# LordLiang/DrawingSpinUp

Hardware: AMD Instinct MI355X
Metric: drawings/sec end-to-end (512x512, 6 views, 24 frames) (higher is better)
Workload: dtype f16 (diffusion) / f16 table + f32 MLP (NSR) / f32 (stage-1 deformable convolutions, IS-Net, contour) / f32 with bf16 x 3 products (stage-2 convolutions; the reference: cuDNN TF32)

## Files before the change

### drawingspinup_amd/csrc/nsr_driver.hip

```cpp
#include "common.h"
#include "adamw_dev.h"

#include <math.h>
#include <string.h>

#include <mutex>
#include <vector>

namespace {

constexpr int N_GEO = 64 * 23 + 64 + 13 * 64 + 13;
constexpr int N_TEX = 64 * 16 + 64 + 64 * 64 + 64 + 3 * 64 + 3;
constexpr int N_SMALL = (64 * 23 + 64 + 64) + (13 * 64 + 13 + 13) + N_TEX + 1;

__device__ __forceinline__ uint4 philox(uint4 c, uint2 k) {
#pragma unroll
  for (int i = 0; i < 10; ++i) {
    const uint32_t hi0 = __umulhi(0xD2511F53u, c.x), lo0 = 0xD2511F53u * c.x;
    const uint32_t hi1 = __umulhi(0xCD9E8D57u, c.z), lo1 = 0xCD9E8D57u * c.z;
    c = make_uint4(hi1 ^ c.y ^ k.x, lo1, hi0 ^ c.w ^ k.y, lo0);
    k.x += 0x9E3779B9u;
    k.y += 0xBB67AE85u;
  }
  return c;
// ... 681 lines not shown
    tex_red.base = L.g_tex;
    have_tex_red = true;
  } else {
    DSU_HIP(hipMemsetAsync(L.d_feat_all, 0, (size_t)(2 * n_r) * 13 * sizeof(float), s));
  }
  DSU_TRY(dsu_sample_losses(L.a_sdf, L.a_grad, n_s, n_r, c.lambda_eikonal, c.lambda_sparsity,
                            c.sparsity_scale, c.lambda_smooth, 1 | 2, L.d_sdf_all, L.d_grad_all,
                            terms + 4, s));
  float* gg = L.g_geo;
  DSU_TRY(mark(d, 1, s));
  DSU_TRY(dsu_sdf_fd_bwd_sorted_fold(&c.grid, a->table_img, &mlp, pts, perm, n_all, c.radius, a->eps,
                                     a->active_levels, L.d_sdf_all, L.d_grad_all, L.d_feat_all, nullptr,
                                     a->table_grad, gg, gg + 64 * 23, gg + 64 * 23 + 64,
                                     gg + 64 * 23 + 64 + 13 * 64, L.sdf_ws, L.sdf_ws_bytes,
                                     L.enc_cache, d->gate, have_tex_red ? &tex_red : nullptr, s));
  DSU_TRY(mark(d, 1, s));
  if (d->timing) { d->work[1] += alg_bytes; d->flops[1] += bwd_flops; }
  DSU_TRY(launch_small_update(d, a, 1, s));
  d->last_step = a->step;
  guard.ok = true;
  return DSU_OK;
}

int dsu_nsr_driver_occ_refresh(dsu_nsr_driver* d, const dsu_occgrid_refresh_args* args,
                               void* main_stream) {
  if (!d || !args) return DSU_EINVAL;
  if (!d->initialised) return DSU_EUNSUP;
  const dsu_nsr_driver_cfg& c = d->cfg;
  DSU_HIP(hipStreamSynchronize(d->side));
  for (int k = 0; k < 3; ++k) d->pf_valid[k] = false;
  dsu_occgrid_refresh_args a = *args;
  const dsu_sdf_mlp mlp{d->L.w0_eff, c.b0, d->L.w1_eff, c.b1};
  a.grid = &c.grid;
  a.mlp = &mlp;
  a.inv_s = d->L.inv_s;
  a.aabb = d->aabb;
  a.seed = c.seed;
  a.radius = c.radius;
  a.render_step_size = c.render_step_size;
  return dsu_occgrid_refresh(&a, main_stream);
}

int dsu_nsr_driver_timing(dsu_nsr_driver* d, int32_t enable) {
  if (!d) return DSU_EINVAL;
  for (int f = 0; f < 2; ++f) {
    for (hipEvent_t e : d->ev[f]) (void)hipEventDestroy(e);
// ... 35 lines not shown
```

### drawingspinup_amd/nsr/encoding.py

```python
import torch
import torch.nn as nn

from .. import ops


class _EncodeFn(torch.autograd.Function):
    @staticmethod
    def forward(ctx, x, params, enc, active):
        ctx.save_for_backward(x)
        ctx.enc, ctx.active = enc, active
        return ops.hashgrid_encode_fwd(enc.cfg, enc.table_f16(), x, active)

    @staticmethod
    def backward(ctx, dout):
        (x,) = ctx.saved_tensors
        g = ops.hashgrid_encode_bwd(ctx.enc.cfg, x, dout.float(), ctx.active)
        return None, g, None, None


_INIT_CACHE = {}


class Encoding(nn.Module):
    def __init__(self, n_input_dims, encoding_config, seed=1337, dtype=None):
# ... 53 lines not shown
    def forward(self, x):
        return _EncodeFn.apply(x.float().contiguous(), self.params, self, self.active_levels)


class ProgressiveBandHashGrid(nn.Module):

    def __init__(self, in_channels, config):
        super().__init__()
        self.n_input_dims = in_channels
        encoding_config = dict(config)
        encoding_config["otype"] = "HashGrid"
        self.encoding = Encoding(in_channels, encoding_config)
        self.n_output_dims = self.encoding.n_output_dims
        self.n_level = config["n_levels"]
        self.n_features_per_level = config["n_features_per_level"]
        self.start_level, self.start_step, self.update_steps = \
            config["start_level"], config["start_step"], config["update_steps"]
        self.current_level = self.start_level
        self.encoding.active_levels = self.current_level

    def forward(self, x):
        return self.encoding(x).float()

    def update_step(self, epoch, global_step):
        self.current_level = min(
            self.start_level + max(global_step - self.start_step, 0) // self.update_steps,
            self.n_level)
        self.encoding.active_levels = self.current_level
```

### drawingspinup_amd/nsr/model.py

```python
import math

import torch
import torch.nn as nn
import torch.nn.functional as F

from .. import ops
from .encoding import ProgressiveBandHashGrid
from .render import (ContractionType, OccupancyGrid, accumulate_along_rays, ray_marching,
                     render_weight_from_alpha)


class Cfg(dict):
    __getattr__ = dict.get

    def __init__(self, d=None, **kw):
        super().__init__()
        for k, v in {**(d or {}), **kw}.items():
            self[k] = Cfg(v) if isinstance(v, dict) else v


DEFAULT_MODEL_CONFIG = Cfg({
    "name": "neus", "radius": 1.0, "num_samples_per_ray": 1024, "train_num_rays": 256,
    "max_train_num_rays": 8192, "grid_prune": True, "grid_prune_occ_thre": 0.001,
    "dynamic_ray_sampling": True, "batch_image_sampling": True, "randomized": True,
# ... 251 lines not shown
                                  self.active_levels, need)
        else:
            with torch.no_grad():
                o = ops.sdf_fd_fwd(enc.cfg, enc.table_f16(),
                                   [t.detach().contiguous() for t in (w0, b0, w1, b1)], pts,
                                   self.radius, eps, self.active_levels, *need)
            outs = [t for t in o if t is not None]
        it = iter(outs)
        rv = [next(it).view(shp), next(it).view(*shp, 3)]
        if with_feature:
            rv.append(next(it).view(*shp, 13))
        if with_laplace:
            rv.append(next(it).view(shp))
        return rv

    @torch.no_grad()
    def forward_level(self, points):
        enc = self.hashgrid
        w = [t.detach().contiguous() for t in self._mlp()]
        pts = points.reshape(-1, 3).float().contiguous()
        return ops.sdf_fwd(enc.cfg, enc.table_f16(), w, pts, self.radius, self.active_levels,
                           1).view(points.shape[:-1])

    def update_step(self, epoch, global_step):
        self.encoding.update_step(epoch, global_step)
        if isinstance(self.finite_difference_eps, float):
            self._finite_difference_eps = self.finite_difference_eps
        elif self.finite_difference_eps == "progressive":
            hg = self.config.xyz_encoding_config
            current_level = min(hg.start_level + max(global_step - hg.start_step, 0)
                                // hg.update_steps, hg.n_levels)
            grid_res = hg.base_resolution * hg.per_level_scale ** (current_level - 1)
            self._finite_difference_eps = 2 * self.config.radius / grid_res
        else:
            raise ValueError(f"Unknown finite_difference_eps={self.finite_difference_eps}")

    def regularizations(self, out):
        return {}


class VolumeRadiance(nn.Module):

    def __init__(self, config):
        super().__init__()
        self.config = config
        self.n_output_dims = 3
        self.n_input_dims = config.input_feature_dim
        self.network = VanillaMLP(self.n_input_dims, 3, dict(config.mlp_network_config))

    def forward(self, features, dirs, *args):
        inp = torch.cat([features.view(-1, features.shape[-1])]
                        + [a.view(-1, a.shape[-1]) for a in args], -1)
        color = self.network(inp).view(*features.shape[:-1], 3).float()
        if "color_activation" in self.config:
            assert self.config.color_activation == "sigmoid"
            color = torch.sigmoid(color)
        return color

# ... 52 lines not shown
        r = config.radius
        self.register_buffer("scene_aabb", torch.as_tensor([-r, -r, -r, r, r, r],
                                                           dtype=torch.float32))
        self._aabb_host = [-r, -r, -r, r, r, r]
        if config.grid_prune:
            self.occupancy_grid = OccupancyGrid(roi_aabb=self._aabb_host, resolution=128,
                                                contraction_type=ContractionType.AABB)
        self.randomized = config.randomized
        self.render_step_size = 1.732 * 2 * config.radius / config.num_samples_per_ray
        self.cos_anneal_ratio = 1.0
        self.fused_shading = True

    def occ_eval_fn(self, x):
        sdf = self.geometry(x, with_grad=False, with_feature=False)
        inv_s = self.variance(torch.zeros([1, 3]))[:, :1].clip(1e-6, 1e6)
        inv_s = inv_s.expand(sdf.shape[0], 1)
        next_sdf = sdf[..., None] - self.render_step_size * 0.5
        prev_sdf = sdf[..., None] + self.render_step_size * 0.5
        prev_cdf = torch.sigmoid(prev_sdf * inv_s)
        next_cdf = torch.sigmoid(next_sdf * inv_s)
        p, c = prev_cdf - next_cdf, prev_cdf
        return ((p + 1e-5) / (c + 1e-5)).view(-1, 1).clip(0.0, 1.0)

    def update_step(self, epoch, global_step):
        self.geometry.update_step(epoch, global_step)
        cos_anneal_end = self.config.get("cos_anneal_end", 0)
        self.cos_anneal_ratio = 1.0 if cos_anneal_end == 0 else min(1.0, global_step / cos_anneal_end)
        if self.training and self.config.grid_prune:
            self.occupancy_grid.every_n_step(step=global_step, occ_eval_fn=self.occ_eval_fn,
                                             occ_thre=self.config.get("grid_prune_occ_thre", 0.01))

    def get_alpha(self, sdf, normal, dirs, dists):
        inv_s = self.variance(torch.zeros([1, 3]))[:, :1].clip(1e-6, 1e6)
        inv_s = inv_s.expand(sdf.shape[0], 1)
        true_cos = (dirs * normal).sum(-1, keepdim=True)
        iter_cos = -(F.relu(-true_cos * 0.5 + 0.5) * (1.0 - self.cos_anneal_ratio)
                     + F.relu(-true_cos) * self.cos_anneal_ratio)
        next_sdf = sdf[..., None] + iter_cos * dists.reshape(-1, 1) * 0.5
        prev_sdf = sdf[..., None] - iter_cos * dists.reshape(-1, 1) * 0.5
        prev_cdf = torch.sigmoid(prev_sdf * inv_s)
        next_cdf = torch.sigmoid(next_sdf * inv_s)
        p, c = prev_cdf - next_cdf, prev_cdf
        return ((p + 1e-5) / (c + 1e-5)).view(-1).clip(0.0, 1.0)

    def forward_(self, rays, jitter=None, pts_random=None, perturb=None):
        n_rays = rays.shape[0]
        rays_o, rays_d = rays[:, 0:3].contiguous(), rays[:, 3:6].contiguous()
        with torch.no_grad():
            ray_indices, t_starts, t_ends = ray_marching(
                rays_o, rays_d, scene_aabb=self._aabb_host,
# ... 117 lines not shown
```

### drawingspinup_amd/nsr/render.py

```python
import enum

import torch
import torch.nn as nn

from .. import ops


class ContractionType(enum.Enum):
    AABB = 0
    UN_BOUNDED_TANH = 1
    UN_BOUNDED_SPHERE = 2


class OccupancyGrid(nn.Module):
    NUM_DIM = 3

    def __init__(self, roi_aabb, resolution=128, contraction_type=ContractionType.AABB):
        super().__init__()
        assert contraction_type == ContractionType.AABB, "only AABB grids are on the hot path"
        if isinstance(resolution, int):
            resolution = [resolution] * 3
        assert resolution[0] == resolution[1] == resolution[2]
        self.res = int(resolution[0])
        self.num_cells = self.res ** 3
        self.contraction_type = contraction_type
        self.register_buffer("_roi_aabb", torch.as_tensor(roi_aabb, dtype=torch.float32))
        self.register_buffer("resolution", torch.tensor(resolution, dtype=torch.int32))
        self.register_buffer("occs", torch.zeros(self.num_cells))
# ... 11 lines not shown
        return self._binary

    def binary_u8(self):
        if self._binary_u8 is None or self._binary_u8.device != self.occs.device:
            self._binary_u8 = self._binary.reshape(-1).to(torch.uint8).contiguous()
        return self._binary_u8

    @torch.no_grad()
    def _cell_points(self, indices, rand=None):
        res = self.res
        if indices is None:
            indices = torch.arange(self.num_cells, device=self.occs.device)
        ix = torch.div(indices, res * res, rounding_mode="floor")
        iy = torch.div(indices, res, rounding_mode="floor") % res
        iz = indices % res
        coords = torch.stack([ix, iy, iz], -1).float()
        if rand is None:
            rand = torch.rand_like(coords)
        x = (coords + rand) / res
        lo, hi = self._roi_aabb[:3], self._roi_aabb[3:]
        return x * (hi - lo) + lo

    @torch.no_grad()
    def _update(self, step, occ_eval_fn, occ_thre=0.01, ema_decay=0.95, warmup_steps=256,
                rand=None, indices=None):
        if (self.native_refresh is not None and rand is None and indices is None
                and self.native_refresh(self, step, step < warmup_steps, occ_thre, ema_decay)):
            return
        if indices is None and step >= warmup_steps:
            n = self.num_cells // 4
            uniform = torch.randint(self.num_cells, (n,), device=self.occs.device)
            occupied = torch.nonzero(self._binary.flatten())[:, 0]
            if n < len(occupied):
                sel = torch.randint(len(occupied), (n,), device=self.occs.device)
                occupied = occupied[sel]
            indices = torch.cat([uniform, occupied], 0)
        x = self._cell_points(indices, rand)
        occ = occ_eval_fn(x).reshape(-1)
        ops.occgrid_ema(self.occs, indices, occ, ema_decay)
        thre = torch.clamp(self.occs.mean(), max=occ_thre)
        self._binary_u8 = ops.occgrid_binarize(self.occs, float(thre))
        self._binary = self._binary_u8.view(self.res, self.res, self.res).bool()

    @torch.no_grad()
    def every_n_step(self, step, occ_eval_fn, occ_thre=1e-2, ema_decay=0.95, warmup_steps=256,
                     n=16):
        if not self.training:
            raise RuntimeError("OccupancyGrid.every_n_step() is a training-only call")
        if step % n == 0:
            self._update(step, occ_eval_fn, occ_thre, ema_decay, warmup_steps)


class RayPacking:
    last = None
    total = 0


@torch.no_grad()
def ray_marching(rays_o, rays_d, t_min=None, t_max=None, scene_aabb=None, grid=None,
                 sigma_fn=None, alpha_fn=None, early_stop_eps=1e-4, alpha_thre=0.0,
                 near_plane=None, far_plane=None, render_step_size=1e-3, stratified=False,
                 cone_angle=0.0, jitter=None):
    assert cone_angle == 0.0 and sigma_fn is None and alpha_fn is None
    aabb = [float(v) for v in scene_aabb.tolist()] if torch.is_tensor(scene_aabb) else scene_aabb
    if stratified and jitter is None:
        jitter = torch.rand(rays_o.shape[0], device=rays_o.device)
    if not stratified:
        jitter = None
    tmin, tmax = ops.ray_aabb(rays_o, rays_d, aabb, jitter, render_step_size)
# ... 64 lines not shown
```

### drawingspinup_amd/nsr/system.py

```python
import math
import os

import numpy as np
import torch
import torch.nn.functional as F

from .. import ops
from .model import Cfg, NeuSModel

DEFAULT_SYSTEM_CONFIG = Cfg({
    "loss": {"lambda_rgb_mse": 0.5, "lambda_rgb_l1": 0.0, "lambda_mask": 1.0,
             "lambda_eikonal": 0.2, "lambda_normal": 1.0, "lambda_3d_normal_smooth": 1.0,
             "lambda_sparsity": 0.5, "sparsity_scale": 100.0, "geo_aware": True,
             "rgb_p_ratio": 0.8, "normal_p_ratio": 0.8, "mask_p_ratio": 0.9},
    "optimizer": {"lr": 0.01, "betas": (0.9, 0.99), "eps": 1e-15,
                  "params": {"geometry": 0.001, "texture": 0.01, "variance": 0.001}},
    "constant_steps": 500, "max_steps": 3000,
})

VIEWS = ["front", "front_right", "right", "back", "left", "front_left"]
_SPATIAL_SORT_BITS = 6

_PACK_CAPACITY = 1 << 19

_AZIMUTH = {"front": 0.0, "front_right": 45.0, "right": 90.0, "back": 180.0, "left": 270.0,
            "front_left": 315.0}


def ideal_w2c(view):
    a = math.radians(_AZIMUTH[view])
    c, s = round(math.cos(a), 12), round(math.sin(a), 12)
# ... 109 lines not shown

    def __float__(self):
        return float(self.detach())

    item = __float__


class TableAdamW:

    def __init__(self, enc, lr, betas, eps, weight_decay=0.01):
        self.enc = enc
        p = enc.params
        self.lr, self.betas, self.eps, self.wd = lr, betas, eps, weight_decay
        self.m = torch.zeros_like(p.data)
        self.v = torch.zeros_like(p.data)
        self.grad = torch.zeros_like(p.data)
        self.step_count = 0
        self.offsets = [2 * o for o in enc.cfg.levels()["offsets"]]
        self.n_levels = enc.cfg.n_levels
        self.active = 0
        self.pending = 1.0
        self.img = None

    def _catch_up(self, upto):
        if upto > self.active:
            a, b = self.offsets[self.active], self.offsets[upto]
            if self.pending != 1.0 and b > a:
                ops.table_decay(self.enc.params.data, self.img, a, b - a, self.pending)
            self.active = upto

    def activate(self, active_levels):
        if self.img is None or self.enc._shadow is not self.img or not self.enc._shadow_locked:
            self.img = self.enc.lock_shadow()
        self._catch_up(max(active_levels, self.active))

    def prepare_step(self, active_levels, lr=None):
        lr = self.lr if lr is None else lr
        if self.img is None or self.enc._shadow is not self.img or not self.enc._shadow_locked:
            self.img = self.enc.lock_shadow()
        if active_levels < self.active:
            active_levels = self.active
        self._catch_up(active_levels)
        b1, b2 = self.betas
        k = self.step_count + 1
        return self.offsets[self.active], lr, 1.0 - b1 ** k, math.sqrt(1.0 - b2 ** k)

    def commit_step(self, lr):
        self.step_count += 1
        self.pending *= 1.0 - lr * self.wd

    def step(self, active_levels, lr=None):
        n, lr, bc1, bc2_sqrt = self.prepare_step(active_levels, lr)
        b1, b2 = self.betas
        ops.table_adamw(self.enc.params.data, self.grad, self.m, self.v, self.img, n, lr, b1, b2,
                        self.eps, self.wd, bc1, bc2_sqrt)
        self.commit_step(lr)

    def finalize(self):
        if self.img is None:
            return
        act = self.active
        self._catch_up(self.n_levels)
        self.active = act
        self.pending = 1.0


class SmallAdamW:

    def __init__(self, torch_optimizer, betas, eps, weight_decay=0.01):
        self.opt = torch_optimizer
        self.betas, self.eps, self.wd = betas, eps, weight_decay
        self.state = {}
        n = sum(len(g["params"]) for g in self.opt.param_groups)
        assert n <= ops._lib.ADAMW_MAX_TENSORS, "more small tensors than dsu_adamw_multi takes"

    def step(self):
        b1, b2 = self.betas
        entries = []
        for group in self.opt.param_groups:
            lr = group["lr"]
            for p in group["params"]:
                g = p.grad
                if g is None:
                    continue
                st = self.state.get(id(p))
                if st is None:
                    st = self.state[id(p)] = [torch.zeros_like(p.data), torch.zeros_like(p.data), 0]
                st[2] += 1
                if not g.is_contiguous():
                    g = g.contiguous()
                entries.append((p.data, g, st[0], st[1], lr, 1.0 - b1 ** st[2],
                                math.sqrt(1.0 - b2 ** st[2])))
        ops.adamw_multi(entries, b1, b2, self.eps, self.wd)


native_timing = {"enabled": False, "totals": {}, "stride": 1}


class NativeStepDriver:

    def __init__(self, system):
        import ctypes as C
        from .. import _lib
        self.C, self._lib = C, _lib
        m, ds, dev = system.model, system.dataset, system.device
        geo = m.geometry
        lin0, lin1 = [l for l in geo.network.layers if isinstance(l, torch.nn.Linear)]
        if not (hasattr(lin0, "weight_g") and m.texture.fused_ok and m.fused_shading):
            raise ops.DsuError("the native step driver is built for the reference networks "
                               "(weight-normed SDF MLP, 16-64-64-3 texture MLP)")
        tensors = (ds.all_c2w, ds.origins, ds.directions, ds.all_images, ds.all_normals_world,
                   ds.all_masks, ds.view_weights)
        if not all(t.is_contiguous() and t.dtype == torch.float32 and t.is_cuda for t in tensors):
            raise ops.DsuError("the native step driver needs the dataset resident as contiguous f32")
        L, oc, mc = system.config.loss, system.config.optimizer, m.config
        c = _lib.NsrDriverCfg()
        c.grid = geo.hashgrid.cfg.c()
        c.radius, c.render_step_size = float(geo.radius), float(m.render_step_size)
        c.cap_points, c.cap_rays = _PACK_CAPACITY, int(mc.max_train_num_rays)
# ... 61 lines not shown
        for fam, name in ((0, "sdf_fd_fwd"), (1, "sdf_fd_bwd")):
            n, ms, work = C.c_int64(), C.c_double(), C.c_double()
            ops.check(self._lib.lib().dsu_nsr_driver_timing_read(
                self.handle, fam, C.byref(n), C.byref(ms), C.byref(work)), "dsu_nsr_driver_timing_read")
            fl = C.c_double()
            ops.check(self._lib.lib().dsu_nsr_driver_timing_flops(self.handle, fam, C.byref(fl)),
                      "dsu_nsr_driver_timing_flops")
            t = native_timing["totals"].setdefault(name, [0, 0.0, 0.0, 0.0])
            t[0] += n.value; t[1] += ms.value; t[2] += work.value; t[3] += fl.value
        ops.check(self._lib.lib().dsu_nsr_driver_timing(self.handle, int(self.timing_on)),
                  "dsu_nsr_driver_timing")

    @property
    def system(self):
        return self._system()

    def occ_refresh(self, grid, step, all_cells, occ_thre, ema_decay, inj_cells=None, inj_rand=None,
                    export=None):
        C, _lib = self.C, self._lib
        if self.handle is None or not self.stepped or self.system is None:
            return False
        if [p._version for p in self.params] != self.param_versions:
            return False
        geo = self.system.model.geometry
        dev = grid.occs.device
        need = int(_lib.lib().dsu_occgrid_refresh_workspace_bytes(grid.res))
        if self._occ_ws is None or self._occ_ws.numel() < need:
            self._occ_ws = torch.empty(need, dtype=torch.uint8, device=dev)
        binary = grid.binary_u8()
        a = _lib.OccRefreshArgs()
        a.occs, a.binary = grid.occs.data_ptr(), binary.data_ptr()
        a.res, a.all_cells = int(grid.res), int(bool(all_cells))
        a.step = int(step)
        a.table_img = geo.hashgrid.table_f16().data_ptr()
        a.active_levels = int(geo.active_levels)
        a.ema_decay, a.occ_thre = float(ema_decay), float(occ_thre)
        keep = []
        if inj_cells is not None:
            ic = inj_cells.to(dev, torch.int32).contiguous()
            ir = inj_rand.to(dev, torch.float32).contiguous()
            keep += [ic, ir]
            a.inj_count, a.inj_cells, a.inj_rand = int(ic.numel()), ic.data_ptr(), ir.data_ptr()
        if export is not None:
            m = int(ic.numel()) if inj_cells is not None else \
                (grid.num_cells if all_cells else 2 * (grid.num_cells // 4))
            export["cells"] = torch.empty(m, dtype=torch.int32, device=dev)
            export["rand"] = torch.empty(m, 3, dtype=torch.float32, device=dev)
            a.cells_out, a.rand_out = export["cells"].data_ptr(), export["rand"].data_ptr()
        a.workspace, a.workspace_bytes = self._occ_ws.data_ptr(), need
        ops.check(_lib.lib().dsu_nsr_driver_occ_refresh(self.handle, C.byref(a), ops.stream()),
                  "dsu_nsr_driver_occ_refresh")
        grid._binary_u8 = binary
        grid._binary = binary.view(grid.res, grid.res, grid.res).bool()
        return True

    def close(self):
        grid = getattr(self.system.model, "occupancy_grid", None) if self.system is not None else None
        if grid is not None and getattr(grid, "native_refresh", None) == self.occ_refresh:
            grid.native_refresh = None
        if self.handle is not None:
            self.flush_timing()
            self._lib.lib().dsu_nsr_driver_destroy(self.handle)
            self.handle = None

    def __del__(self):
        try:
            self.close()
        except Exception:
            pass


class OrthoNeuSSystem:
    def __init__(self, model_config=None, system_config=None, device="cuda", seed=123456):
        torch.manual_seed(seed)
        np.random.seed(seed)
        self.device = torch.device(device)
        self.model = NeuSModel(model_config).to(self.device)
# ... 7 lines not shown
        self.table_opt = None
        self.keep_table_grad = False
        if self.device.type == "cuda":
            self.table_opt = TableAdamW(enc, dict(oc.params)["geometry"], tuple(oc.betas), oc.eps)
            self.model.register_state_dict_pre_hook(lambda *a, **k: self.table_opt.finalize())
        groups = [{"params": [p for p in getattr(self.model, n).parameters()
                              if self.table_opt is None or p is not enc.params],
                   "name": n, "lr": lr}
                  for n, lr in oc.params.items()]
        fused = self.device.type == "cuda"
        self.optimizer = torch.optim.AdamW(groups, lr=oc.lr, betas=tuple(oc.betas), eps=oc.eps,
                                           **({"fused": True} if fused else {}))
        self._base_lrs = [g["lr"] for g in groups]
        self.small_opt = None
        if self.device.type == "cuda":
            self.small_opt = SmallAdamW(self.optimizer, tuple(oc.betas), oc.eps)
        decay_steps = self.config.max_steps - self.config.constant_steps
        self._gamma = 0.1 ** (1.0 / decay_steps) if decay_steps > 0 else 1.0
        self.dataset = None
        self.last = {}
        self.step_mode = "native"
        self.native_with_injected_draws = False
        self._native, self._python_steps = None, 0
        self.fused_batch = True

    def preprocess_data(self, index=None, x=None, y=None):
        ds, n = self.dataset, self.train_num_rays
        dev = self.device
        if index is None:
            index = torch.randint(0, len(ds.all_masks), size=(n,), device=dev)
            x = torch.randint(0, ds.w, size=(n,), device=dev)
            y = torch.randint(0, ds.h, size=(n,), device=dev)
        if self.device.type == "cuda" and self.fused_batch and ds.all_images.dtype == torch.float32 \
                and all(t.is_contiguous() for t in (ds.all_images, ds.all_normals_world,
                                                    ds.all_masks, ds.view_weights, ds.origins,
                                                    ds.directions, ds.all_c2w)):
            return ops.ortho_ray_batch(index, x, y, ds.all_c2w, ds.origins, ds.directions,
                                       ds.all_images, ds.all_normals_world, ds.all_masks,
                                       ds.view_weights)
        return self.preprocess_data_torch(index, x, y)

    def preprocess_data_torch(self, index, x, y):
        ds = self.dataset
        c2w = ds.all_c2w[index]
        directions, origins = ds.directions[index, y, x], ds.origins[index, y, x]
        rays_o, rays_d = get_ortho_rays(origins, directions, c2w)
# ... 33 lines not shown
        lm = ranking_loss_masked(binary_cross_entropy(opac, batch["mask"].float()),
                                 torch.ones_like(mask), L.mask_p_ratio, view_weights)
        terms["mask"] = lm * (L.lambda_mask if self.dataset.has_mask else 0.0)
        return terms

    def sample_losses(self, out):
        L = self.config.loss
        terms = {}
        terms["eikonal"] = ((torch.linalg.norm(out["sdf_grad_samples"], ord=2, dim=-1) - 1.0) ** 2
                            ).mean() * L.lambda_eikonal
        terms["sparsity"] = torch.exp(-L.sparsity_scale * out["random_sdf"].abs()).mean() \
            * L.lambda_sparsity
        if L.lambda_3d_normal_smooth > 0:
            terms["normal_smooth"] = (out["random_sdf_grad"] - out["normal_perturb"]).abs().mean() \
                * L.lambda_3d_normal_smooth
        return terms

    def losses(self, out, batch):
        comp = out.get("comp_raw")
        if comp is None:
            comp = torch.cat([out["opacity"], out["depth"], out["comp_rgb"], out["comp_normal"]], 1)
        return {**self.ray_losses(comp, batch), **self.sample_losses(out)}

    def _set_lr(self):
        s = self.global_step
        f = 1.0 if s < self.config.constant_steps else self._gamma ** (s - self.config.constant_steps)
        for g, base in zip(self.optimizer.param_groups, self._base_lrs):
            g["lr"] = base * f

    def zero_grad(self):
        self.optimizer.zero_grad(set_to_none=True)
        self.model.geometry.hashgrid.params.grad = None

    def _step_small(self):
        if self.small_opt is not None:
            self.small_opt.step()
        else:
            self.optimizer.step()

    def _step_table(self, active_levels):
        if self.table_opt is None:
            self.model.geometry.hashgrid.invalidate()
            return
        lr = next(g["lr"] for g in self.optimizer.param_groups if g.get("name") == "geometry")
        if self.keep_table_grad:
            self.model.geometry.hashgrid.params.grad = self.table_opt.grad.clone()
        self.table_opt.step(int(active_levels), lr)

    def training_step(self, inject=None):
        fusable = self.model.fused_shading and self.train_num_rays <= ops.RAY_LOSS_MAX_RAYS
        native_ok = (self.step_mode == "native" and fusable and self.device.type == "cuda"
# ... 24 lines not shown
        inject = inject or {}
        keep = []
        batch = inject.get("batch") or {}
        for field, key in (("inj_rays", "rays"), ("inj_rgb", "rgb"), ("inj_normal", "normal"),
                           ("inj_mask", "mask"), ("inj_cosines", "cosines"),
                           ("inj_view_weights", "view_weights")):
            t = batch.get(key)
            if t is not None:
                t = t.to(self.device, torch.float32).contiguous()
                keep.append(t)
            setattr(a, field, None if t is None else t.data_ptr())
        if batch and int(batch["rays"].shape[0]) != int(self.train_num_rays):
            raise ValueError("injected ray batch: train_num_rays must equal its row count")
        for field, key, dt in (("inj_index", "index", torch.int64), ("inj_x", "x", torch.int64),
                               ("inj_y", "y", torch.int64), ("inj_jitter", "jitter", torch.float32),
                               ("inj_pts_random", "pts_random", torch.float32),
                               ("inj_perturb", "perturb", torch.float32)):
            t = inject.get(key)
            if t is not None:
                t = t.to(self.device, dt).contiguous()
                keep.append(t)
            setattr(a, field, None if t is None else t.data_ptr())
        nxt = self.global_step + 1
        a.step, a.n_rays = self.global_step, int(self.train_num_rays)
        a.prefetch_next = int(not inject and not (m.config.grid_prune and nxt % 16 == 0))
        a.active_levels, a.eps = int(geo.active_levels), float(geo._finite_difference_eps)
        a.cos_anneal_ratio = float(m.cos_anneal_ratio)
        self._set_lr()
        lrs = {g.get("name"): g["lr"] for g in self.optimizer.param_groups}
        a.lr_geometry, a.lr_texture, a.lr_variance = lrs["geometry"], lrs["texture"], lrs["variance"]
        a.adam_step = drv.adam_step + 1
        a.randomized = int(bool(m.randomized))
        versions = [p._version for p in drv.params]
        a.refresh_effective = int(versions != drv.param_versions)
        drv.param_versions = versions
        if m.config.grid_prune:
            occ = m.occupancy_grid.binary_u8()
            a.occ_binary, a.occ_res = occ.data_ptr(), m.occupancy_grid.res
        else:
            a.occ_binary, a.occ_res = None, 0
        topt = self.table_opt
        topt.activate(int(geo.active_levels))
        n_tab, lr_tab, bc1, bc2s = topt.prepare_step(int(geo.active_levels), lrs["geometry"])
        a.table_img, a.table_grad = topt.img.data_ptr(), topt.grad.data_ptr()
        a.table_p, a.table_m, a.table_v = enc.params.data_ptr(), topt.m.data_ptr(), topt.v.data_ptr()
        if self.keep_table_grad:
            a.table_p = None
        a.table_n, a.table_lr, a.table_bc1, a.table_bc2_sqrt = int(n_tab), lr_tab, bc1, bc2s
        a.table_eps, a.table_wd = float(topt.eps), float(topt.wd)
        terms_copy = torch.empty(8, dtype=torch.float32, device=self.device)
        a.terms_out = terms_copy.data_ptr()
        for attempt in range(6):
            rc = drv._lib.lib().dsu_nsr_driver_step(drv.handle, C.byref(a), ops.stream())
            if rc != -3 or a.out_n_samples <= _PACK_CAPACITY or a.n_rays <= 64:
                break
            a.n_rays = max(64, a.n_rays // 2)
            self.train_num_rays = int(a.n_rays)
        if rc != 0:
            raise ops.DsuError(f"dsu_nsr_driver_step failed ({rc}): {a.out_n_samples} samples, "
                               f"longest ray {a.out_max_count} (capacity {_PACK_CAPACITY})")
        drv.adam_step += 1
        drv.stepped = True
        n_rays = int(self.train_num_rays)
        if m.config.dynamic_ray_sampling:
            self.train_num_rays = int(a.out_next_n_rays)
        if self.keep_table_grad:
            enc.params.grad = topt.grad.clone()
        else:
            topt.commit_step(lr_tab)
        self.global_step += 1
        t = terms_copy
        L = self.config.loss
        terms = {"rgb_mse": t[0]}
        if L.lambda_rgb_l1:
            terms["rgb_l1"] = t[1]
        terms.update({"normal": t[2], "mask": t[3], "eikonal": t[4], "sparsity": t[5]})
        if L.lambda_3d_normal_smooth > 0:
            terms["normal_smooth"] = t[6]
        self.last = {"loss": _LazyLoss(t[0:4], t[4:7]), "n_samples": int(a.out_n_samples),
                     "n_rays": n_rays, **terms}
        return self.last

    def training_step_fused(self, inject=None):
        from .render import RayPacking
        m, L = self.model, self.config.loss
        geo, enc = m.geometry, m.geometry.hashgrid
        m.train()
        inject = inject or {}
        m.update_step(0, self.global_step)
        if self.table_opt is not None:
            self.table_opt.activate(int(geo.active_levels))
        batch = inject.get("batch") or \
            self.preprocess_data(inject.get("index"), inject.get("x"), inject.get("y"))
        rays = batch["rays"]
        rays_o, rays_d = rays[:, 0:3].contiguous(), rays[:, 3:6].contiguous()
        dev = rays_d.device
        n_rays = rays_d.shape[0]
        jitter = inject.get("jitter")
        if jitter is None and m.randomized:
            jitter = torch.rand(n_rays, device=dev)
        with torch.no_grad():
            tmin, tmax = ops.ray_aabb(rays_o, rays_d, m._aabb_host,
                                      jitter if m.randomized else None, m.render_step_size)
            occ, res = None, 0
# ... 125 lines not shown
        from .render import RayPacking
        n_samples = RayPacking.total
        if self.model.config.dynamic_ray_sampling and n_samples > 0:
            tr = int(self.train_num_rays * (self.train_num_samples / n_samples))
            self.train_num_rays = min(int(self.train_num_rays * 0.9 + tr * 0.1),
                                      self.model.config.max_train_num_rays)
        self._set_lr()
        self.zero_grad()
        terms = self.losses(out, batch)
        loss = sum(terms.values())
        loss.backward()
        self._step_small()
        enc = self.model.geometry.hashgrid
        if self.table_opt is not None:
            if enc.params.grad is not None:
                self.table_opt.grad.copy_(enc.params.grad.reshape(-1))
            enc.params.grad = None
        self._step_table(self.model.geometry.active_levels)
        self.global_step += 1
        self.last = {"loss": loss.detach(), "n_samples": n_samples,
                     "n_rays": batch["rays"].shape[0], **{k: v.detach() for k, v in terms.items()}}
        return self.last

    def fit(self, dataset, max_steps=None, log_every=0):
        self.dataset = dataset
        for _ in range(max_steps or self.config.max_steps):
            r = self.training_step()
            if log_every and self.global_step % log_every == 0:
                print(f"[nsr] step {self.global_step} loss {float(r['loss']):.4f} "
                      f"rays {r['n_rays']} samples {r['n_samples']}", flush=True)
        if self.table_opt is not None:
            self.table_opt.finalize()
        if self._native is not None:
            self._native.flush_timing()

    @torch.no_grad()
    def export_mesh(self, front_mask=None, resolution=None, with_colors=True, face_count=None):
        from . import mesh as M
        if self.table_opt is not None:
            self.table_opt.finalize()
        self.model.eval()
        fine, coarse = M.isosurface(self.model, front_mask, resolution, face_count)
        fine["coarse_level"] = coarse["level"]
        fine["vert_colors"] = M.vertex_colors(self.model, fine["verts"].to(self.device)) \
            if with_colors and fine["verts"].shape[0] else None
        return fine

    def export_name(self, front_cutting=True):
        iso = self.model.config.geometry.isosurface
# ... 11 lines not shown
```

### include/dsu_hip.h

```cpp
#ifndef DSU_HIP_H
#define DSU_HIP_H

#include <stdint.h>

#ifdef __cplusplus
extern "C" {
#endif

#define DSU_OK 0
#define DSU_EINVAL (-1)
#define DSU_ELAUNCH (-2)
#define DSU_EUNSUP (-3)

#define DSU_MAX_LEVELS 16

const char* dsu_strerror(int code);
#define DSU_ABI_VERSION 3
int dsu_abi_version(void);
int dsu_set_onewave_grid_cap(int32_t cus);
int dsu_set_scatter_grid_cap(int32_t workgroups);
int dsu_set_nsr_side_stream_priority(int32_t level);
int dsu_set_nsr_side_stream_pooling(int32_t on);

typedef struct {
// ... 422 lines not shown
  float *table_p, *table_m, *table_v;
  int64_t table_n;
  float table_lr, table_bc1, table_bc2_sqrt, table_eps, table_wd;
  int32_t out_n_samples, out_max_count, out_next_n_rays;
  float* terms_out;
} dsu_nsr_step_args;

int dsu_nsr_draws(uint64_t seed, int64_t step, int32_t n_rays, int32_t V, int32_t H, int32_t W,
                  int64_t* index, int64_t* x, int64_t* y, float* jitter, int32_t n_random,
                  float* pts_random, float* perturb, void* stream);
int64_t dsu_nsr_driver_workspace_bytes(const dsu_nsr_driver_cfg* cfg);
int dsu_nsr_driver_create(const dsu_nsr_driver_cfg* cfg, dsu_nsr_driver** out);
void dsu_nsr_driver_destroy(dsu_nsr_driver* d);
int dsu_nsr_driver_step(dsu_nsr_driver* d, dsu_nsr_step_args* args, void* main_stream);
const float* dsu_nsr_driver_terms(const dsu_nsr_driver* d);
const uint32_t* dsu_nsr_driver_live_halves(const dsu_nsr_driver* d, int64_t step);
const float* dsu_nsr_driver_adam_moments(const dsu_nsr_driver* d, int32_t second);
int dsu_nsr_driver_timing(dsu_nsr_driver* d, int32_t enable);
int dsu_nsr_driver_timing_read(dsu_nsr_driver* d, int32_t family, int64_t* launches,
                               double* total_ms, double* alg_bytes);
int dsu_nsr_driver_timing_flops(dsu_nsr_driver* d, int32_t family, double* mlp_flops);
int dsu_nsr_driver_occ_refresh(dsu_nsr_driver* d, const dsu_occgrid_refresh_args* args,
                               void* main_stream);

int32_t dsu_smooth_energy_partials(void);
int dsu_smooth_iterate(const int32_t* nbr, int64_t nv, const double* lower, const double* upper,
                       double weight, int32_t iters, double* x, double* y, void* stream);
int dsu_smooth_energy(const int32_t* nbr, int64_t nv, const double* x, double* y,
                      double* partials, void* stream);

int32_t dsu_smooth_brick_side(void);
int dsu_smooth_bricks_flags(const uint8_t* band, int32_t X, int32_t Y, int32_t Z, int32_t* flags,
                            void* stream);
int dsu_smooth_bricks_gather(const uint8_t* band, const double* dist, int32_t X, int32_t Y, int32_t Z,
                             const int32_t* table, const int32_t* bcoord, int32_t nb,
                             const double* values, int32_t nvalues, double* x, double* x0,
                             uint8_t* code, uint64_t* mask, int32_t* nbr6, int32_t* miss,
                             void* stream);
int dsu_smooth_bricks_iterate(const int32_t* nbr6, const uint64_t* mask, int32_t nb, const double* x0,
                              const uint8_t* code, const double* values, int32_t nvalues,
                              double weight, int32_t iters, int32_t direct, double* x, double* y,
                              void* stream);
int dsu_smooth_bricks_energy(const int32_t* nbr6, const uint64_t* mask, int32_t nb, const double* x,
                             double* partials, void* stream);
int dsu_smooth_bricks_scatter(const double* x, const uint64_t* mask, const int32_t* bcoord, int32_t nb,
                              int32_t X, int32_t Y, int32_t Z, double* dist, void* stream);
// ... 215 lines not shown
```

Before: 0.3781.

## Run the whole NSR training loop natively from a precomputed schedule

After: 0.3815, median of 2. About the same (+0.9%).

```diff
diff --git a/drawingspinup_amd/csrc/nsr_driver.hip b/drawingspinup_amd/csrc/nsr_driver.hip
--- a/drawingspinup_amd/csrc/nsr_driver.hip
+++ b/drawingspinup_amd/csrc/nsr_driver.hip
@@ -727,6 +727,84 @@
   return DSU_OK;
 }
 
+int dsu_nsr_driver_fit(dsu_nsr_driver* d, const dsu_nsr_step_args* first, const double* schedule,
+                       int64_t n_steps, const dsu_occgrid_refresh_args* refresh,
+                       int32_t refresh_every, int64_t refresh_warmup_steps, double* trace,
+                       float* terms_out, int64_t* out, void* main_stream) {
+  if (!d || !first || !out || n_steps < 0 || (n_steps && !schedule) || (refresh && refresh_every < 1) ||
+      !first->table_p || !first->table_img)
+    return DSU_EINVAL;
+  if (first->inj_index || first->inj_x || first->inj_y || first->inj_jitter || first->inj_pts_random ||
+      first->inj_perturb || first->inj_rays)
+    return DSU_EINVAL;
+  if (!d->initialised) return DSU_EUNSUP;
+  dsu_nsr_step_args a = *first;
+  a.terms_out = nullptr;
+  out[0] = 0; out[1] = a.n_rays; out[2] = 0; out[3] = 0; out[4] = -1; out[5] = 0; out[6] = 0; out[7] = 0;
+  for (int64_t i = 0; i < n_steps; ++i) {
+    const double* row = schedule + i * DSU_NSR_FIT_COLS;
+    const int64_t step = first->step + i;
+    a.step = step;
+    a.adam_step = first->adam_step + (int32_t)i;
+    if (i) a.refresh_effective = 0;
+    a.active_levels = (uint32_t)row[0];
+    a.eps = (float)row[1];
+    a.cos_anneal_ratio = (float)row[2];
+    a.lr_geometry = (float)row[3]; a.lr_texture = (float)row[4]; a.lr_variance = (float)row[5];
+    a.table_n = (int64_t)row[6];
+    a.table_lr = (float)row[7]; a.table_bc1 = (float)row[8]; a.table_bc2_sqrt = (float)row[9];
+    int rc = DSU_OK;
+    bool refreshed = false;
+    if (refresh && step % refresh_every == 0) {
+      dsu_occgrid_refresh_args r = *refresh;
+      r.step = step;
+      r.all_cells = step < refresh_warmup_steps ? 1 : 0;
+      r.active_levels = a.active_levels;
+      rc = dsu_nsr_driver_occ_refresh(d, &r, main_stream);
+      if (rc == DSU_OK) { refreshed = true; ++out[6]; }
+    }
+    const int64_t dec_start = (int64_t)row[10], dec_n = (int64_t)row[11];
+    if (rc == DSU_OK && dec_n > 0) {
+      if (dec_start < 0) rc = DSU_EINVAL;
+      else rc = dsu_table_decay(a.table_p + dec_start, (char*)const_cast<void*>(a.table_img) + 2 * dec_start,
+                                dec_n, (float)row[12], main_stream);
+      if (rc == DSU_OK) ++out[5];
+    }
+    a.prefetch_next = (refresh && (step + 1) % refresh_every == 0) ? 0 : 1;
+    a.terms_out = i == n_steps - 1 ? terms_out : nullptr;
+    int attempts = 0;
+    while (rc == DSU_OK) {
+      rc = dsu_nsr_driver_step(d, &a, main_stream);
+      ++attempts;
+      if (rc != DSU_EUNSUP || attempts >= 6 || a.out_n_samples <= d->cfg.cap_points || a.n_rays <= 64) break;
+      a.n_rays = a.n_rays / 2 > 64 ? a.n_rays / 2 : 64;
+      rc = DSU_OK;
+    }
+    if (rc != DSU_OK) {
+      out[1] = a.n_rays;
+      out[4] = step;
+      out[7] = a.out_max_count;
+      return rc;
+    }
+    if (trace) {
+      double* t = trace + i * DSU_NSR_FIT_TRACE_COLS;
+      t[0] = (double)step; t[1] = refreshed ? 1.0 : 0.0; t[2] = (double)a.prefetch_next;
+      t[3] = (double)a.n_rays; t[4] = (double)a.out_n_samples; t[5] = (double)a.out_next_n_rays;
+      t[6] = (double)a.adam_step; t[7] = (double)attempts;
+      t[8] = (double)a.active_levels; t[9] = (double)a.eps; t[10] = (double)a.cos_anneal_ratio;
+      t[11] = (double)a.lr_geometry; t[12] = (double)a.lr_texture; t[13] = (double)a.lr_variance;
+      t[14] = (double)a.table_n; t[15] = (double)a.table_lr; t[16] = (double)a.table_bc1;
+      t[17] = (double)a.table_bc2_sqrt; t[18] = row[10]; t[19] = row[11]; t[20] = (double)(float)row[12];
+    }
+    out[0] = i + 1;
+    out[2] = a.out_n_samples;
+    out[3] = a.n_rays;
+    a.n_rays = a.out_next_n_rays;
+    out[1] = a.n_rays;
+  }
+  return DSU_OK;
+}
+
 int dsu_nsr_driver_occ_refresh(dsu_nsr_driver* d, const dsu_occgrid_refresh_args* args,
                                void* main_stream) {
   if (!d || !args) return DSU_EINVAL;
diff --git a/drawingspinup_amd/nsr/encoding.py b/drawingspinup_amd/nsr/encoding.py
--- a/drawingspinup_amd/nsr/encoding.py
+++ b/drawingspinup_amd/nsr/encoding.py
@@ -99,8 +99,10 @@
     def forward(self, x):
         return self.encoding(x).float()
 
+    def level_at(self, global_step):
+        return min(self.start_level + max(global_step - self.start_step, 0) // self.update_steps,
+                   self.n_level)
+
     def update_step(self, epoch, global_step):
-        self.current_level = min(
-            self.start_level + max(global_step - self.start_step, 0) // self.update_steps,
-            self.n_level)
+        self.current_level = self.level_at(global_step)
         self.encoding.active_levels = self.current_level
diff --git a/drawingspinup_amd/nsr/model.py b/drawingspinup_amd/nsr/model.py
--- a/drawingspinup_amd/nsr/model.py
+++ b/drawingspinup_amd/nsr/model.py
@@ -297,18 +297,20 @@
         return ops.sdf_fwd(enc.cfg, enc.table_f16(), w, pts, self.radius, self.active_levels,
                            1).view(points.shape[:-1])
 
-    def update_step(self, epoch, global_step):
-        self.encoding.update_step(epoch, global_step)
+    def eps_at(self, global_step):
         if isinstance(self.finite_difference_eps, float):
-            self._finite_difference_eps = self.finite_difference_eps
-        elif self.finite_difference_eps == "progressive":
+            return self.finite_difference_eps
+        if self.finite_difference_eps == "progressive":
             hg = self.config.xyz_encoding_config
             current_level = min(hg.start_level + max(global_step - hg.start_step, 0)
                                 // hg.update_steps, hg.n_levels)
             grid_res = hg.base_resolution * hg.per_level_scale ** (current_level - 1)
-            self._finite_difference_eps = 2 * self.config.radius / grid_res
-        else:
-            raise ValueError(f"Unknown finite_difference_eps={self.finite_difference_eps}")
+            return 2 * self.config.radius / grid_res
+        raise ValueError(f"Unknown finite_difference_eps={self.finite_difference_eps}")
+
+    def update_step(self, epoch, global_step):
+        self.encoding.update_step(epoch, global_step)
+        self._finite_difference_eps = self.eps_at(global_step)
 
     def regularizations(self, out):
         return {}
@@ -407,10 +409,16 @@
         p, c = prev_cdf - next_cdf, prev_cdf
         return ((p + 1e-5) / (c + 1e-5)).view(-1, 1).clip(0.0, 1.0)
 
+    def cos_anneal_at(self, global_step):
+        cos_anneal_end = self.config.get("cos_anneal_end", 0)
+        return 1.0 if cos_anneal_end == 0 else min(1.0, global_step / cos_anneal_end)
+
+    def set_schedule(self, global_step):
+        self.geometry.update_step(0, global_step)
+        self.cos_anneal_ratio = self.cos_anneal_at(global_step)
+
     def update_step(self, epoch, global_step):
-        self.geometry.update_step(epoch, global_step)
-        cos_anneal_end = self.config.get("cos_anneal_end", 0)
-        self.cos_anneal_ratio = 1.0 if cos_anneal_end == 0 else min(1.0, global_step / cos_anneal_end)
+        self.set_schedule(global_step)
         if self.training and self.config.grid_prune:
             self.occupancy_grid.every_n_step(step=global_step, occ_eval_fn=self.occ_eval_fn,
                                              occ_thre=self.config.get("grid_prune_occ_thre", 0.01))
diff --git a/drawingspinup_amd/nsr/render.py b/drawingspinup_amd/nsr/render.py
--- a/drawingspinup_amd/nsr/render.py
+++ b/drawingspinup_amd/nsr/render.py
@@ -4,6 +4,8 @@
 import torch.nn as nn
 
 from .. import ops
+
+REFRESH_EVERY, WARMUP_STEPS, EMA_DECAY = 16, 256, 0.95
 
 
 class ContractionType(enum.Enum):
@@ -61,7 +63,7 @@
         return x * (hi - lo) + lo
 
     @torch.no_grad()
-    def _update(self, step, occ_eval_fn, occ_thre=0.01, ema_decay=0.95, warmup_steps=256,
+    def _update(self, step, occ_eval_fn, occ_thre=0.01, ema_decay=EMA_DECAY, warmup_steps=WARMUP_STEPS,
                 rand=None, indices=None):
         if (self.native_refresh is not None and rand is None and indices is None
                 and self.native_refresh(self, step, step < warmup_steps, occ_thre, ema_decay)):
@@ -82,8 +84,8 @@
         self._binary = self._binary_u8.view(self.res, self.res, self.res).bool()
 
     @torch.no_grad()
-    def every_n_step(self, step, occ_eval_fn, occ_thre=1e-2, ema_decay=0.95, warmup_steps=256,
-                     n=16):
+    def every_n_step(self, step, occ_eval_fn, occ_thre=1e-2, ema_decay=EMA_DECAY,
+                     warmup_steps=WARMUP_STEPS, n=REFRESH_EVERY):
         if not self.training:
             raise RuntimeError("OccupancyGrid.every_n_step() is a training-only call")
         if step % n == 0:
diff --git a/drawingspinup_amd/nsr/system.py b/drawingspinup_amd/nsr/system.py
--- a/drawingspinup_amd/nsr/system.py
+++ b/drawingspinup_amd/nsr/system.py
@@ -7,6 +7,7 @@
 
 from .. import ops
 from .model import Cfg, NeuSModel
+from .render import EMA_DECAY, REFRESH_EVERY, WARMUP_STEPS
 
 DEFAULT_SYSTEM_CONFIG = Cfg({
     "loss": {"lambda_rgb_mse": 0.5, "lambda_rgb_l1": 0.0, "lambda_mask": 1.0,
@@ -162,22 +163,27 @@
         self.pending = 1.0
         self.img = None
 
+    def _ensure_image(self):
+        if self.img is None or self.enc._shadow is not self.img or not self.enc._shadow_locked:
+            self.img = self.enc.lock_shadow()
+
+    def _decay(self, start, n, factor):
+        ops.table_decay(self.enc.params.data, self.img, start, n, factor)
+
     def _catch_up(self, upto):
         if upto > self.active:
             a, b = self.offsets[self.active], self.offsets[upto]
             if self.pending != 1.0 and b > a:
-                ops.table_decay(self.enc.params.data, self.img, a, b - a, self.pending)
+                self._decay(a, b - a, self.pending)
             self.active = upto
 
     def activate(self, active_levels):
-        if self.img is None or self.enc._shadow is not self.img or not self.enc._shadow_locked:
-            self.img = self.enc.lock_shadow()
+        self._ensure_image()
         self._catch_up(max(active_levels, self.active))
 
     def prepare_step(self, active_levels, lr=None):
         lr = self.lr if lr is None else lr
-        if self.img is None or self.enc._shadow is not self.img or not self.enc._shadow_locked:
-            self.img = self.enc.lock_shadow()
+        self._ensure_image()
         if active_levels < self.active:
             active_levels = self.active
         self._catch_up(active_levels)
@@ -203,6 +209,25 @@
         self._catch_up(self.n_levels)
         self.active = act
         self.pending = 1.0
+
+
+class TableSchedule(TableAdamW):
+
+    def __init__(self, offsets, lr, betas, wd=0.01, step_count=0, active=0, pending=1.0):
+        self.lr, self.betas, self.wd = lr, betas, wd
+        self.offsets, self.n_levels = list(offsets), len(offsets) - 1
+        self.step_count, self.active, self.pending = step_count, active, pending
+        self.events = []
+
+    @classmethod
+    def of(cls, opt):
+        return cls(opt.offsets, opt.lr, opt.betas, opt.wd, opt.step_count, opt.active, opt.pending)
+
+    def _ensure_image(self):
+        pass
+
+    def _decay(self, start, n, factor):
+        self.events.append((start, n, factor))
 
 
 class SmallAdamW:
@@ -235,6 +260,8 @@
 
 
 native_timing = {"enabled": False, "totals": {}, "stride": 1}
+
+_SCHEDULE_CACHE = {}
 
 
 class NativeStepDriver:
@@ -342,19 +369,8 @@
             return False
         if [p._version for p in self.params] != self.param_versions:
             return False
-        geo = self.system.model.geometry
         dev = grid.occs.device
-        need = int(_lib.lib().dsu_occgrid_refresh_workspace_bytes(grid.res))
-        if self._occ_ws is None or self._occ_ws.numel() < need:
-            self._occ_ws = torch.empty(need, dtype=torch.uint8, device=dev)
-        binary = grid.binary_u8()
-        a = _lib.OccRefreshArgs()
-        a.occs, a.binary = grid.occs.data_ptr(), binary.data_ptr()
-        a.res, a.all_cells = int(grid.res), int(bool(all_cells))
-        a.step = int(step)
-        a.table_img = geo.hashgrid.table_f16().data_ptr()
-        a.active_levels = int(geo.active_levels)
-        a.ema_decay, a.occ_thre = float(ema_decay), float(occ_thre)
+        a, binary = self.refresh_args(grid, step, all_cells, occ_thre, ema_decay)
         keep = []
         if inj_cells is not None:
             ic = inj_cells.to(dev, torch.int32).contiguous()
@@ -367,12 +383,28 @@
             export["cells"] = torch.empty(m, dtype=torch.int32, device=dev)
             export["rand"] = torch.empty(m, 3, dtype=torch.float32, device=dev)
             a.cells_out, a.rand_out = export["cells"].data_ptr(), export["rand"].data_ptr()
-        a.workspace, a.workspace_bytes = self._occ_ws.data_ptr(), need
         ops.check(_lib.lib().dsu_nsr_driver_occ_refresh(self.handle, C.byref(a), ops.stream()),
                   "dsu_nsr_driver_occ_refresh")
         grid._binary_u8 = binary
         grid._binary = binary.view(grid.res, grid.res, grid.res).bool()
         return True
+
+    def refresh_args(self, grid, step, all_cells, occ_thre, ema_decay):
+        _lib = self._lib
+        geo = self.system.model.geometry
+        need = int(_lib.lib().dsu_occgrid_refresh_workspace_bytes(grid.res))
+        if self._occ_ws is None or self._occ_ws.numel() < need:
+            self._occ_ws = torch.empty(need, dtype=torch.uint8, device=grid.occs.device)
+        binary = grid.binary_u8()
+        a = _lib.OccRefreshArgs()
+        a.occs, a.binary = grid.occs.data_ptr(), binary.data_ptr()
+        a.res, a.all_cells = int(grid.res), int(bool(all_cells))
+        a.step = int(step)
+        a.table_img = geo.hashgrid.table_f16().data_ptr()
+        a.active_levels = int(geo.active_levels)
+        a.ema_decay, a.occ_thre = float(ema_decay), float(occ_thre)
+        a.workspace, a.workspace_bytes = self._occ_ws.data_ptr(), need
+        return a, binary
 
     def close(self):
         grid = getattr(self.system.model, "occupancy_grid", None) if self.system is not None else None
@@ -426,6 +458,7 @@
         self.step_mode = "native"
         self.native_with_injected_draws = False
         self._native, self._python_steps = None, 0
+        self.keep_fit_trace, self.fit_trace = False, None
         self.fused_batch = True
 
     def preprocess_data(self, index=None, x=None, y=None):
@@ -505,11 +538,62 @@
             comp = torch.cat([out["opacity"], out["depth"], out["comp_rgb"], out["comp_normal"]], 1)
         return {**self.ray_losses(comp, batch), **self.sample_losses(out)}
 
-    def _set_lr(self):
-        s = self.global_step
-        f = 1.0 if s < self.config.constant_steps else self._gamma ** (s - self.config.constant_steps)
+    def _lr_factor(self, s):
+        return 1.0 if s < self.config.constant_steps else self._gamma ** (s - self.config.constant_steps)
+
+    def _set_lr(self, step=None):
+        f = self._lr_factor(self.global_step if step is None else step)
         for g, base in zip(self.optimizer.param_groups, self._base_lrs):
             g["lr"] = base * f
+
+    def step_scalars(self, step):
+        m, f = self.model, self._lr_factor(step)
+        lrs = {g.get("name"): base * f for g, base in zip(self.optimizer.param_groups, self._base_lrs)}
+        return {"active_levels": int(m.geometry.encoding.encoding.level_at(step)),
+                "eps": float(m.geometry.eps_at(step)),
+                "cos_anneal_ratio": float(m.cos_anneal_at(step)),
+                "lr_geometry": lrs["geometry"], "lr_texture": lrs["texture"],
+                "lr_variance": lrs["variance"]}
+
+    def fit_schedule(self, first_step, n_steps, table=None):
+        from .. import _lib
+        key = None
+        if table is None:
+            table = TableSchedule.of(self.table_opt)
+            key = (first_step, n_steps, self._schedule_inputs(), tuple(table.offsets), table.lr,
+                   tuple(table.betas), table.wd, table.step_count, table.active, table.pending)
+            hit = _SCHEDULE_CACHE.get("latest")
+            if hit is not None and hit[0] == key:
+                return hit[1], hit[2]
+        rows = np.zeros((n_steps, _lib.DEFINES["DSU_NSR_FIT_COLS"]), np.float64)
+        states = []
+        for i in range(n_steps):
+            sc = self.step_scalars(first_step + i)
+            seen = len(table.events)
+            table.activate(sc["active_levels"])
+            n_tab, lr_tab, bc1, bc2s = table.prepare_step(sc["active_levels"], sc["lr_geometry"])
+            table.commit_step(lr_tab)
+            rows[i, :10] = (sc["active_levels"], sc["eps"], sc["cos_anneal_ratio"], sc["lr_geometry"],
+                            sc["lr_texture"], sc["lr_variance"], n_tab, lr_tab, bc1, bc2s)
+            new = table.events[seen:]
+            assert len(new) <= 1
+            if new:
+                rows[i, 10:13] = new[0]
+            states.append((table.step_count, table.pending, table.active))
+        if key is not None:
+            rows.setflags(write=False)
+            _SCHEDULE_CACHE["latest"] = (key, rows, states)
+        return rows, states
+
+    def _schedule_inputs(self):
+        m, geo = self.model, self.model.geometry
+        hg, gc = geo.encoding.encoding, geo.config.xyz_encoding_config
+        return (self.config.constant_steps, self._gamma, tuple(self._base_lrs),
+                tuple(g.get("name") for g in self.optimizer.param_groups),
+                hg.start_level, hg.start_step, hg.update_steps, hg.n_level,
+                geo.finite_difference_eps, geo.config.radius, gc.start_level, gc.start_step,
+                gc.update_steps, gc.n_levels, gc.base_resolution, gc.per_level_scale,
+                m.config.get("cos_anneal_end", 0))
 
     def zero_grad(self):
         self.optimizer.zero_grad(set_to_none=True)
@@ -580,13 +664,13 @@
                 keep.append(t)
             setattr(a, field, None if t is None else t.data_ptr())
         nxt = self.global_step + 1
+        sc = self.step_scalars(self.global_step)
         a.step, a.n_rays = self.global_step, int(self.train_num_rays)
-        a.prefetch_next = int(not inject and not (m.config.grid_prune and nxt % 16 == 0))
-        a.active_levels, a.eps = int(geo.active_levels), float(geo._finite_difference_eps)
-        a.cos_anneal_ratio = float(m.cos_anneal_ratio)
+        a.prefetch_next = int(not inject and not (m.config.grid_prune and nxt % REFRESH_EVERY == 0))
+        a.active_levels, a.eps = sc["active_levels"], sc["eps"]
+        a.cos_anneal_ratio = sc["cos_anneal_ratio"]
         self._set_lr()
-        lrs = {g.get("name"): g["lr"] for g in self.optimizer.param_groups}
-        a.lr_geometry, a.lr_texture, a.lr_variance = lrs["geometry"], lrs["texture"], lrs["variance"]
+        a.lr_geometry, a.lr_texture, a.lr_variance = sc["lr_geometry"], sc["lr_texture"], sc["lr_variance"]
         a.adam_step = drv.adam_step + 1
         a.randomized = int(bool(m.randomized))
         versions = [p._version for p in drv.params]
@@ -598,8 +682,8 @@
         else:
             a.occ_binary, a.occ_res = None, 0
         topt = self.table_opt
-        topt.activate(int(geo.active_levels))
-        n_tab, lr_tab, bc1, bc2s = topt.prepare_step(int(geo.active_levels), lrs["geometry"])
+        topt.activate(sc["active_levels"])
+        n_tab, lr_tab, bc1, bc2s = topt.prepare_step(sc["active_levels"], sc["lr_geometry"])
         a.table_img, a.table_grad = topt.img.data_ptr(), topt.grad.data_ptr()
         a.table_p, a.table_m, a.table_v = enc.params.data_ptr(), topt.m.data_ptr(), topt.v.data_ptr()
         if self.keep_table_grad:
@@ -627,7 +711,10 @@
         else:
             topt.commit_step(lr_tab)
         self.global_step += 1
-        t = terms_copy
+        self.last = self._native_result(terms_copy, int(a.out_n_samples), n_rays)
+        return self.last
+
+    def _native_result(self, t, n_samples, n_rays):
         L = self.config.loss
         terms = {"rgb_mse": t[0]}
         if L.lambda_rgb_l1:
@@ -635,9 +722,7 @@
         terms.update({"normal": t[2], "mask": t[3], "eikonal": t[4], "sparsity": t[5]})
         if L.lambda_3d_normal_smooth > 0:
             terms["normal_smooth"] = t[6]
-        self.last = {"loss": _LazyLoss(t[0:4], t[4:7]), "n_samples": int(a.out_n_samples),
-                     "n_rays": n_rays, **terms}
-        return self.last
+        return {"loss": _LazyLoss(t[0:4], t[4:7]), "n_samples": n_samples, "n_rays": n_rays, **terms}
 
     def training_step_fused(self, inject=None):
         from .render import RayPacking
@@ -809,9 +894,78 @@
                      "n_rays": batch["rays"].shape[0], **{k: v.detach() for k, v in terms.items()}}
         return self.last
 
+    def _fit_loop_ok(self):
+        drv = self._native
+        return (drv is not None and drv.handle is not None and drv.stepped and drv.dataset is self.dataset
+                and self.step_mode == "native" and not self.keep_table_grad and self.table_opt is not None
+                and self.train_num_rays <= ops.RAY_LOSS_MAX_RAYS
+                and [p._version for p in drv.params] == drv.param_versions)
+
+    def _fit_native(self, n_steps):
+        import ctypes as C
+        drv, m, topt = self._native, self.model, self.table_opt
+        geo, enc, lib = m.geometry, m.geometry.hashgrid, self._native._lib
+        first = int(self.global_step)
+        rows, states = self.fit_schedule(first, n_steps)
+        m.train()
+        a = drv.args
+        for field in ("inj_rays", "inj_rgb", "inj_normal", "inj_mask", "inj_cosines", "inj_view_weights",
+                      "inj_index", "inj_x", "inj_y", "inj_jitter", "inj_pts_random", "inj_perturb"):
+            setattr(a, field, None)
+        a.step, a.n_rays = first, int(self.train_num_rays)
+        a.adam_step, a.randomized, a.refresh_effective = drv.adam_step + 1, int(bool(m.randomized)), 0
+        refresh, binary = None, None
+        if m.config.grid_prune:
+            grid = m.occupancy_grid
+            r, binary = drv.refresh_args(grid, first, False, m.config.get("grid_prune_occ_thre", 0.01),
+                                         EMA_DECAY)
+            refresh = C.byref(r)
+            a.occ_binary, a.occ_res = binary.data_ptr(), grid.res
+        else:
+            a.occ_binary, a.occ_res = None, 0
+        topt._ensure_image()
+        a.table_img, a.table_grad = topt.img.data_ptr(), topt.grad.data_ptr()
+        a.table_p, a.table_m, a.table_v = enc.params.data_ptr(), topt.m.data_ptr(), topt.v.data_ptr()
+        a.table_eps, a.table_wd = float(topt.eps), float(topt.wd)
+        terms = torch.empty(8, dtype=torch.float32, device=self.device)
+        out = (C.c_int64 * lib.DEFINES["DSU_NSR_FIT_OUT"])()
+        trace = None
+        if self.keep_fit_trace:
+            trace = np.full((n_steps, lib.DEFINES["DSU_NSR_FIT_TRACE_COLS"]), np.nan, np.float64)
+        rc = lib.lib().dsu_nsr_driver_fit(
+            drv.handle, C.byref(a), rows.ctypes.data, n_steps, refresh, REFRESH_EVERY, WARMUP_STEPS,
+            None if trace is None else trace.ctypes.data, terms.data_ptr(), C.addressof(out), ops.stream())
+        done, events = int(out[0]), int(out[5])
+        if done:
+            topt.step_count, topt.pending, topt.active = states[done - 1]
+            drv.adam_step += done
+            self.global_step = first + done
+            m.set_schedule(self.global_step - 1)
+            self._set_lr(self.global_step - 1)
+            self.last = self._native_result(terms, int(out[2]), int(out[3]))
+        if events > int(np.count_nonzero(rows[:done, 11])):
+            topt.active = states[done][2]
+        self.train_num_rays = int(out[1])
+        if binary is not None and out[6]:
+            grid._binary_u8 = binary
+            grid._binary = binary.view(grid.res, grid.res, grid.res).bool()
+        if trace is not None:
+            self.fit_trace = {"trace": trace[:done], "schedule": rows, "first_step": first}
+        if rc != 0:
+            raise ops.DsuError(f"dsu_nsr_driver_fit failed ({rc}) at step {int(out[4])}: "
+                               f"{int(a.out_n_samples)} samples, longest ray {int(out[7])} "
+                               f"(capacity {_PACK_CAPACITY})")
+
     def fit(self, dataset, max_steps=None, log_every=0):
         self.dataset = dataset
-        for _ in range(max_steps or self.config.max_steps):
+        n = max_steps or self.config.max_steps
+        if not log_every and n > 0:
+            self.training_step()
+            n -= 1
+            if n > 0 and self._fit_loop_ok():
+                self._fit_native(n)
+                n = 0
+        for _ in range(n):
             r = self.training_step()
             if log_every and self.global_step % log_every == 0:
                 print(f"[nsr] step {self.global_step} loss {float(r['loss']):.4f} "
diff --git a/include/dsu_hip.h b/include/dsu_hip.h
--- a/include/dsu_hip.h
+++ b/include/dsu_hip.h
@@ -468,6 +468,13 @@
 int dsu_nsr_driver_timing_flops(dsu_nsr_driver* d, int32_t family, double* mlp_flops);
 int dsu_nsr_driver_occ_refresh(dsu_nsr_driver* d, const dsu_occgrid_refresh_args* args,
                                void* main_stream);
+#define DSU_NSR_FIT_COLS 13
+#define DSU_NSR_FIT_TRACE_COLS 21
+#define DSU_NSR_FIT_OUT 8
+int dsu_nsr_driver_fit(dsu_nsr_driver* d, const dsu_nsr_step_args* first, const double* schedule,
+                       int64_t n_steps, const dsu_occgrid_refresh_args* refresh,
+                       int32_t refresh_every, int64_t refresh_warmup_steps, double* trace,
+                       float* terms_out, int64_t* out, void* main_stream);
 
 int32_t dsu_smooth_energy_partials(void);
 int dsu_smooth_iterate(const int32_t* nbr, int64_t nv, const double* lower, const double* upper,
```
